# TXH-mercury/VALOR

Measured on AMD Instinct MI355X. Metric: pretrain samples/sec (V+A+T clip), higher is better.
Workload: dtype bf16

## Files before the change

valor_amd/csrc/gemm.hip:

```cpp
#include "gemm_common.h"
#include <stdlib.h>

template <typename T, bool TA, bool TB>
__global__ __launch_bounds__(256) void gemm_kernel(GemmArgs p) {
    constexpr int VEC = ElemTraits<T>::VEC;
    constexpr int BK = 8 * VEC;
    constexpr int TILE_BYTES = 128 * TILE_ROW_BYTES;
    extern __shared__ __attribute__((aligned(16))) char smem[];

    const int tid = threadIdx.x;
    const int lane = tid & 63;
    const int wave = __builtin_amdgcn_readfirstlane(tid >> 6);
    const int wm = wave >> 1, wn = wave & 1;

    const int tiles_n = (p.N + 127) >> 7;
    const int tiles_m = (p.M + 127) >> 7;
    const int logical = xcd_remap(blockIdx.x, tiles_m * tiles_n);
    const int tm = logical / tiles_n, tn = logical - tm * tiles_n;
    const int m0 = tm << 7, n0 = tn << 7;

    const int nk_total = (p.K + BK - 1) / BK;
    int ks_begin = 0, ks_end = nk_total;
    if (p.kslices > 1) {
        ks_begin = blockIdx.y * p.ksteps_per_slice;
// ... 329 lines not shown
    }
}

template <typename T>
DEVINL void splitk_reduce_body(const GemmArgs& p, int bid, int nblk) {
    if (p.ws_bf16 && (p.N & 7) == 0) {
        const int64_t noct = (int64_t)p.N >> 3, total8 = (int64_t)p.M * noct, sl = (int64_t)p.M * p.N;
        for (int64_t i = (int64_t)bid * blockDim.x + threadIdx.x; i < total8; i += (int64_t)nblk * blockDim.x) {
            const int m = (int)(i / noct);
            const int n = (int)(i - (int64_t)m * noct) << 3;
            const bf16_t* q = (const bf16_t*)p.ws + (int64_t)m * p.N + n;
            f32x4_t s0 = {0.f, 0.f, 0.f, 0.f}, s1 = s0;
            auto add = [&](const u32x4_t r) {
                s0 += (f32x4_t){__uint_as_float(r[0] << 16), __uint_as_float(r[0] & 0xffff0000u), __uint_as_float(r[1] << 16), __uint_as_float(r[1] & 0xffff0000u)};
                s1 += (f32x4_t){__uint_as_float(r[2] << 16), __uint_as_float(r[2] & 0xffff0000u), __uint_as_float(r[3] << 16), __uint_as_float(r[3] & 0xffff0000u)};
            };
            int k = 0;
            for (; k + 4 <= p.kslices; k += 4) {
                const u32x4_t r0 = *(const u32x4_t*)(q + (int64_t)k * sl), r1 = *(const u32x4_t*)(q + (int64_t)(k + 1) * sl);
                const u32x4_t r2 = *(const u32x4_t*)(q + (int64_t)(k + 2) * sl), r3 = *(const u32x4_t*)(q + (int64_t)(k + 3) * sl);
                add(r0); add(r1); add(r2); add(r3);
            }
            for (; k < p.kslices; ++k) add(*(const u32x4_t*)(q + (int64_t)k * sl));
            epilogue_store<T>(p, m, n, s0, load_bias4<T>(p, n));
            epilogue_store<T>(p, m, n + 4, s1, load_bias4<T>(p, n + 4));
        }
    } else {
    const int64_t nquads = ((int64_t)p.N + 3) >> 2;
    const int64_t total = (int64_t)p.M * nquads;
    for (int64_t i = (int64_t)bid * blockDim.x + threadIdx.x; i < total; i += (int64_t)nblk * blockDim.x) {
        const int m = (int)(i / nquads);
        const int n = (int)(i - (int64_t)m * nquads) << 2;
        f32x4_t s = {0.f, 0.f, 0.f, 0.f};
        if (p.ws_bf16) {
            for (int k = 0; k < p.kslices; ++k) {
                const bf16_t* q = (const bf16_t*)p.ws + ((int64_t)k * p.M + m) * p.N + n;
                if (n + 3 < p.N && (p.N & 3) == 0) s += load4<bf16_t>(q);
                else for (int r = 0; r < 4; ++r) if (n + r < p.N) s[r] += (float)q[r];
            }
        } else {
            for (int k = 0; k < p.kslices; ++k) {
                const float* q = p.ws + ((int64_t)k * p.M + m) * p.N + n;
                if (n + 3 < p.N && (p.N & 3) == 0) s += *(const f32x4_t*)q;
                else for (int r = 0; r < 4; ++r) if (n + r < p.N) s[r] += q[r];
            }
        }
        epilogue_store<T>(p, m, n, s, load_bias4<T>(p, n));
    }
    }
    if (p.rowsum_out) {
        for (int m = bid * blockDim.x + threadIdx.x; m < p.M; m += nblk * blockDim.x) {
            float t = 0.f;
            for (int k = 0; k < p.kslices; ++k) t += p.rowsum_ws[(int64_t)k * p.M + m];
            rowsum_store<T>(p, m, t);
        }
    }
}
template <typename T>
__global__ __launch_bounds__(256) void gemm_splitk_reduce(GemmArgs p) {
    splitk_reduce_body<T>(p, blockIdx.x, gridDim.x);
}

#define VALOR_REDUCE_GROUP 8
struct ReduceGroupArgs {
    GemmArgs g[VALOR_REDUCE_GROUP];
    int first[VALOR_REDUCE_GROUP + 1];
    int n;
};
template <typename T>
__global__ __launch_bounds__(256) void gemm_splitk_reduce_group(ReduceGroupArgs a) {
    int i = 0;
    while (i + 1 < a.n && (int)blockIdx.x >= a.first[i + 1]) ++i;
    splitk_reduce_body<T>(a.g[i], blockIdx.x - a.first[i], a.first[i + 1] - a.first[i]);
}
static int reduce_blocks(const GemmArgs& p) {
    const int64_t total = (int64_t)p.M * ((p.N + 3) / 4);
    int blocks = (int)((total + 255) / 256);
    return blocks > 4096 ? 4096 : blocks;
}

static int g_gemm_variant = 4;
static inline int gemm_variant() { return GEMM_KNOB(variant, g_gemm_variant); }
extern "C" int valor_gemm_set_variant(int v) { const int o = g_gemm_variant; if (v >= 0 && v <= 4) g_gemm_variant = v; return o; }
thread_local const GemmTuning* t_gemm_tuning = nullptr;
int g_gemm_policy_default[13] = {[] { const char* e = getenv("VALOR_GEMM_NT_MINK"); return e ? atoi(e) : 768; }(),
                        [] { const char* e = getenv("VALOR_GEMM_SPLITK_BF16"); return e ? atoi(e) : 1; }(),
                        [] { const char* e = getenv("VALOR_GEMM_MIN_TILES"); return e ? atoi(e) : 256; }(),
                        [] { const char* e = getenv("VALOR_GEMM_NT_MIN_TILES"); return e ? atoi(e) : 1024; }(),
                        [] { const char* e = getenv("VALOR_GEMM_RASTER"); return e ? atoi(e) : 1000; }(),
                        [] { const char* e = getenv("VALOR_GEMM_STORE"); return e ? atoi(e) : 1000; }(),
                        [] { const char* e = getenv("VALOR_GEMM_NTA"); return e ? atoi(e) : 0; }(),
                        [] { const char* e = getenv("VALOR_GEMM_NN_MINK"); return e ? atoi(e) : 128; }(),
                        [] { const char* e = getenv("VALOR_GEMM_NARROW"); return e ? atoi(e) : 1000; }(),
                        [] { const char* e = getenv("VALOR_GEMM_MFMA32"); return e ? atoi(e) : 0; }(),
                        [] { const char* e = getenv("VALOR_GEMM_WIDE"); return e ? atoi(e) : 0; }(),
                        [] { const char* e = getenv("VALOR_GEMM_SKINNY_ALL"); return e ? atoi(e) : 0; }(),
                        [] { const char* e = getenv("VALOR_GEMM_WAVE128"); return e ? atoi(e) : 1000; }()};
extern "C" int valor_gemm_set_policy(int key, int value) {
    if (key < 0 || key > 12) return VALOR_ERR_ARG;
    const int old = g_gemm_policy_default[key];
    if (value >= 0) g_gemm_policy_default[key] = value;
    return old;
}

static bool use_8ph(int dtype, int transA, int transB, int M, int N, int K, bool heavy_epi = false) {
    if (dtype != VALOR_DT_BF16 || gemm_variant() < 3) return false;
    if ((K % 64) != 0 || K < 128 || M < 256 || N < 256) return false;
    if (gemm_variant() == 3) return true;
    const int64_t tiles256 = (int64_t)((M + 255) / 256) * ((N + 255) / 256);
    if (transA && transB) return K >= 4096;
    if (!transA && !transB) return tiles256 >= gemm_policy(2) && K >= gemm_policy(7);
    if (!transA && transB) return tiles256 >= gemm_policy(3) && K >= (heavy_epi ? 1536 : gemm_policy(0));
    return false;
}

static bool use_8ph2(int dtype, int transA, int transB, int M, int N, int K, bool heavy_epi, bool big) {
    const int mode = gemm_policy(8);
    if (dtype != VALOR_DT_BF16 || gemm_variant() != 4 || mode == 0) return false;
    if ((K % 64) != 0 || K < 128 || M < 256 || N < 128) return false;
    if (transA && !transB) return false;
    if (mode == 1) return true;
    if (mode == 2) return !big;
    if (mode == 3) return big;
    (void)heavy_epi;
    if (transA) return false;
    if (!big) return true;
    const int64_t tiles256 = (int64_t)((M + 255) / 256) * ((N + 255) / 256);
    return K <= 1024 && (N >= 1536 || tiles256 < 1024);
}

static int gemm_family(int dtype, int transA, int transB, int M, int N, int K, bool heavy_epi) {
    if (dtype != VALOR_DT_BF16 || gemm_variant() == 0) return 0;
    if (gemm_variant() == 4 && !transA && !transB && M <= gemm_policy(11) && N >= 16 && gemm_skinny_chunks(K)) return 5;
    const bool big = use_8ph(dtype, transA, transB, M, N, K, heavy_epi);
    if (use_8ph2(dtype, transA, transB, M, N, K, heavy_epi, big)) return 4;
    if (big) return 3;
    return gemm_variant() == 2 ? 2 : 1;
}

static int family3_ktiles_per_workgroup(int M, int N, int K) {
    const int nk = K / 64, tiles = ((M + 255) / 256) * ((N + 255) / 256);
    int sl = 1;
    if (2 * tiles <= 256 && nk >= 24) {
        sl = 256 / tiles;
        if (sl > nk / 6) sl = nk / 6;
        if (sl > 64) sl = 64;
        if (sl < 2) sl = 1;
    }
    return (nk + sl - 1) / sl;
}
static bool use_wave128(int dtype, int transA, int transB, int M, int N, int K, bool heavy_epi) {
    const int mode = gemm_policy(12);
    if (mode == 0 || gemm_family(dtype, transA, transB, M, N, K, heavy_epi) != 3) return false;
    if (!(transA && transB)) return false;
    if (mode == 1) return true;
    return family3_ktiles_per_workgroup(M, N, K) > 48;
}
extern "C" int valor_gemm_wave128_for(int dtype, int transA, int transB, int M, int N, int K, int heavy_epilogue) {
    return use_wave128(dtype, transA, transB, M, N, K, heavy_epilogue != 0) ? 1 : 0;
}

extern "C" int valor_gemm_kernel_for(int dtype, int transA, int transB, int M, int N, int K, int heavy_epilogue) {
    return gemm_family(dtype, transA, transB, M, N, K, heavy_epilogue != 0);
}
struct TuningScope {
    const GemmTuning* prev;
    explicit TuningScope(const void* t) : prev(t_gemm_tuning) { if (t) t_gemm_tuning = (const GemmTuning*)t; }
    ~TuningScope() { t_gemm_tuning = prev; }
};
static_assert(sizeof(GemmTuning) == 17 * sizeof(int), "valor_gemm_policy layout (include/valor_hip.h)");
extern "C" int valor_gemm_kernel_for_tuned(const void* policy, int dtype, int transA, int transB, int M, int N, int K, int heavy_epilogue) {
    TuningScope scope(policy);
    return gemm_family(dtype, transA, transB, M, N, K, heavy_epilogue != 0);
}

template <int NSTAGE>
static void launch_gemm_glds(hipStream_t st, int transA, int transB, const GemmArgs& p, dim3 grid) {
    const size_t lds = NSTAGE * 32768;
#define VALOR_GLDS_LAUNCH1(TA_, TB_, F_, W_)                                                        \
    do {                                                                                            \
        static bool attr_set = false;                                                               \
        if (!attr_set) {                                                                            \
            hipFuncSetAttribute((const void*)gemm_glds_kernel<TA_, TB_, NSTAGE, F_, W_>,            \
                                hipFuncAttributeMaxDynamicSharedMemorySize, (int)lds);              \
            attr_set = true;                                                                        \
        }                                                                                           \
        hipLaunchKernelGGL((gemm_glds_kernel<TA_, TB_, NSTAGE, F_, W_>), grid, dim3(256), lds, st, p); \
    } while (0)
#define VALOR_GLDS_LAUNCH(TA_, TB_)                                                                 \
    do {                                                                                            \
        if constexpr (NSTAGE == 1) {                                                                \
            if (fused) VALOR_GLDS_LAUNCH1(TA_, TB_, true, 3);                                       \
            else VALOR_GLDS_LAUNCH1(TA_, TB_, false, 4);                                            \
        } else {                                                                                    \
            if (fused) VALOR_GLDS_LAUNCH1(TA_, TB_, true, 2);                                       \
            else VALOR_GLDS_LAUNCH1(TA_, TB_, false, 2);                                            \
        }                                                                                           \
    } while (0)
    const bool fused = p.kslices <= 1 && ((p.act & VALOR_ACT_MASK) != VALOR_ACT_NONE || p.preact || p.dact_aux);
    if (!transA && !transB) VALOR_GLDS_LAUNCH(false, false);
    else if (!transA && transB) VALOR_GLDS_LAUNCH(false, true);
    else if (transA && !transB) VALOR_GLDS_LAUNCH(true, false);
    else VALOR_GLDS_LAUNCH(true, true);
#undef VALOR_GLDS_LAUNCH
#undef VALOR_GLDS_LAUNCH1
}

template <typename T>
static int launch_gemm(hipStream_t st, int transA, int transB, GemmArgs p) {
    const int tiles = ((p.M + 127) / 128) * ((p.N + 127) / 128);
    dim3 grid(tiles, p.kslices > 1 ? p.kslices : 1);
    if (ElemTraits<T>::DT == VALOR_DT_BF16 && gemm_variant() > 0) {
        if (p.kslices > 1) grid = dim3(tiles * p.kslices, 1);
        const int fam = gemm_family(VALOR_DT_BF16, transA, transB, p.M, p.N, p.K, p.dact_aux != nullptr && !(p.act & VALOR_ACT_DERIV));
        if (fam == 4) launch_gemm_8ph2(st, transA, transB, p);
        else if (fam == 3) {
            if (use_wave128(VALOR_DT_BF16, transA, transB, p.M, p.N, p.K, p.dact_aux != nullptr && !(p.act & VALOR_ACT_DERIV))) launch_gemm_8q(st, transA, transB, p);
            else launch_gemm_8ph(st, transA, transB, p);
        } else {
            p.st_mode = (gemm_policy(6) && !p.out_f32 && p.kslices <= 1 && p.K <= 1024 && (int64_t)p.M * p.N >= (4 << 20)) ? 1 : 0;
            if (gemm_variant() == 2) launch_gemm_glds<2>(st, transA, transB, p, grid);
            else launch_gemm_glds<1>(st, transA, transB, p, grid);
        }
        if (p.kslices > 1 && !p.defer_reduce)
            hipLaunchKernelGGL((gemm_splitk_reduce<T>), dim3(reduce_blocks(p)), dim3(256), 0, st, p);
        return valor_launch_status();
    }
    const size_t lds = 2 * 2 * 128 * TILE_ROW_BYTES;
#define VALOR_GEMM_LAUNCH(TA_, TB_)                                                               \
    do {                                                                                          \
        static bool attr_set = false;                                                             \
        if (!attr_set) {                                                                          \
            hipFuncSetAttribute((const void*)gemm_kernel<T, TA_, TB_>,                            \
                                hipFuncAttributeMaxDynamicSharedMemorySize, (int)lds);            \
            attr_set = true;                                                                      \
        }                                                                                         \
        hipLaunchKernelGGL((gemm_kernel<T, TA_, TB_>), grid, dim3(256), lds, st, p);              \
    } while (0)
    if (!transA && !transB) VALOR_GEMM_LAUNCH(false, false);
    else if (!transA && transB) VALOR_GEMM_LAUNCH(false, true);
    else if (transA && !transB) VALOR_GEMM_LAUNCH(true, false);
    else VALOR_GEMM_LAUNCH(true, true);
#undef VALOR_GEMM_LAUNCH
    if (p.kslices > 1 && !p.defer_reduce)
        hipLaunchKernelGGL((gemm_splitk_reduce<T>), dim3(reduce_blocks(p)), dim3(256), 0, st, p);
    return valor_launch_status();
}

struct PendingBlob { GemmArgs p; int dtype; int valid; };
static_assert(sizeof(PendingBlob) <= 256, "valor_gemm_pending is 256 bytes");

static int gemm_impl(void* stream, int dtype, int transA, int transB, int M, int N, int K,
                     const void* A, int64_t lda, const void* B, int64_t ldb, void* C, int64_t ldc,
                     const void* bias, int act, void* preact, const void* dact_aux, int64_t ldaux,
                     float alpha, int accumulate, int out_f32, void* workspace, int64_t workspace_bytes,
                     void* rowsum_out, int rowsum_accumulate, PendingBlob* pending);

extern "C" int valor_gemm(void* stream, int dtype, int transA, int transB, int M, int N, int K,
                          const void* A, int64_t lda, const void* B, int64_t ldb, void* C, int64_t ldc,
                          const void* bias, int act, void* preact, const void* dact_aux, int64_t ldaux,
                          float alpha, int accumulate, int out_f32, void* workspace, int64_t workspace_bytes,
                          void* rowsum_out, int rowsum_accumulate) {
    return gemm_impl(stream, dtype, transA, transB, M, N, K, A, lda, B, ldb, C, ldc, bias, act, preact, dact_aux, ldaux, alpha, accumulate,
                     out_f32, workspace, workspace_bytes, rowsum_out, rowsum_accumulate, nullptr);
}

extern "C" int valor_gemm_tuned(const void* policy, void* stream, int dtype, int transA, int transB, int M, int N, int K,
                                const void* A, int64_t lda, const void* B, int64_t ldb, void* C, int64_t ldc,
                                const void* bias, int act, void* preact, const void* dact_aux, int64_t ldaux,
                                float alpha, int accumulate, int out_f32, void* workspace, int64_t workspace_bytes,
                                void* rowsum_out, int rowsum_accumulate) {
    TuningScope scope(policy);
    return gemm_impl(stream, dtype, transA, transB, M, N, K, A, lda, B, ldb, C, ldc, bias, act, preact, dact_aux, ldaux, alpha, accumulate,
                     out_f32, workspace, workspace_bytes, rowsum_out, rowsum_accumulate, nullptr);
}

extern "C" int valor_gemm_deferred(void* stream, int dtype, int transA, int transB, int M, int N, int K,
                                   const void* A, int64_t lda, const void* B, int64_t ldb, void* C, int64_t ldc,
                                   const void* bias, int act, void* preact, const void* dact_aux, int64_t ldaux,
                                   float alpha, int accumulate, int out_f32, void* workspace, int64_t workspace_bytes,
                                   void* rowsum_out, int rowsum_accumulate, void* pending) {
    if (!pending) return VALOR_ERR_ARG;
    PendingBlob* pb = (PendingBlob*)pending;
    pb->valid = 0; pb->dtype = dtype; pb->p.kslices = 0;
    return gemm_impl(stream, dtype, transA, transB, M, N, K, A, lda, B, ldb, C, ldc, bias, act, preact, dact_aux, ldaux, alpha, accumulate,
                     out_f32, workspace, workspace_bytes, rowsum_out, rowsum_accumulate, pb);
}

extern "C" int valor_gemm_pending_bytes(const void* pending, int64_t* bytes) {
    if (!pending || !bytes) return VALOR_ERR_ARG;
    const PendingBlob* pb = (const PendingBlob*)pending;
    *bytes = 0;
    if (!pb->valid || pb->p.kslices <= 1) return VALOR_OK;
    const int64_t n = ((int64_t)pb->p.kslices * pb->p.M * pb->p.N + (int64_t)pb->p.kslices * pb->p.M) * 4;
    *bytes = (n + 255) & ~(int64_t)255;
    return VALOR_OK;
}

extern "C" int valor_gemm_reduce_group(void* stream, int dtype, const void* pendings, int n) {
    if (n <= 0) return VALOR_OK;
    if (!pendings || n > VALOR_REDUCE_GROUP) return VALOR_ERR_ARG;
    ReduceGroupArgs a;
    a.n = 0; a.first[0] = 0;
    for (int i = 0; i < n; ++i) {
        const PendingBlob* pb = (const PendingBlob*)((const char*)pendings + (size_t)i * 256);
        if (!pb->valid || pb->p.kslices <= 1) continue;
        if (pb->dtype != dtype) return VALOR_ERR_ARG;
        a.g[a.n] = pb->p;
// ... 123 lines not shown
```

valor_amd/csrc/gemm8.hip:

```cpp
#include "gemm_common.h"
#include <stdlib.h>

#define HT_BYTES 16384
#define BUF_BYTES (4 * HT_BYTES)
#define OFF_A0 0
#define OFF_A1 HT_BYTES
#define OFF_B0 (2 * HT_BYTES)
#define OFF_B1 (3 * HT_BYTES)

DEVINL bf16x8_t read_frag_tr8(const char* img, int off, int kk) {
    const char* a = img + off + kk * (32 * 256);
    s16x4_t lo = lds_read_tr4(a), hi = lds_read_tr4(a + 4 * 256);
    return __builtin_bit_cast(bf16x8_t, __builtin_shufflevector(lo, hi, 0, 1, 2, 3, 4, 5, 6, 7));
}

template <bool TA, bool TB, bool ASMTR, bool NTS = false, int SCHED = 0>
__global__ __launch_bounds__(512, 2) void gemm_8ph_kernel(GemmArgs p) {
    typedef bf16_t T;
    constexpr int BK = 64;
    extern __shared__ __attribute__((aligned(16))) char smem[];

    const int tid = threadIdx.x;
    const int lane = tid & 63;
    const int wave = __builtin_amdgcn_readfirstlane(tid >> 6);
// ... 349 lines not shown
        }
    }

    if constexpr (!TA) if (p.fast_epi) {
        char* sB = smem;
        const int act = p.act & VALOR_ACT_MASK;
        const bool deriv = (p.act & VALOR_ACT_DERIV) != 0;
        auto write_tile = [&](bool apply_act) {
#pragma unroll
            for (int ni = 0; ni < 4; ++ni) {
                const int col = (ni >> 1) * 128 + wn * 32 + (ni & 1) * 16 + 4 * fg;
                const f32x4_t bias4 = load_bias4<T>(p, n0 + col);
#pragma unroll
                for (int mi = 0; mi < 8; ++mi) {
                    const int row = (mi >> 2) * 128 + wm * 64 + (mi & 3) * 16 + fr;
                    f32x4_t v = acc[mi][ni];
#pragma unroll
                    for (int r = 0; r < 4; ++r) v[r] = v[r] * p.alpha + bias4[r];
                    if (apply_act) {
                        float f[4] = {v[0], v[1], v[2], v[3]};
                        act_fwd_n<4>(act, f);
                        v = (f32x4_t){f[0], f[1], f[2], f[3]};
                    }
                    const u32x2_t w = {pack2_bf16(v[0], v[1]), pack2_bf16(v[2], v[3])};
                    *(u32x2_t*)(sB + row * 512 + (((col >> 3) ^ (row & 31)) << 4) + (fg & 1) * 8) = w;
                }
            }
        };
        auto read_tile = [&](T* dst) {
#pragma unroll 4
            for (int it = 0; it < 16; ++it) {
                const int ml = it * 16 + (tid >> 5), c = tid & 31;
                const u32x4_t val = *(const u32x4_t*)(sB + ml * 512 + ((c ^ (ml & 31)) << 4));
                const int m = m0 + ml, n = n0 + c * 8;
                if (m < p.M && n < p.N) store_out16<NTS>(dst + (int64_t)m * p.ldc + n, val);
            }
        };
        if (p.preact) {
            write_tile(false);
            __syncthreads();
            read_tile((T*)p.preact);
            __syncthreads();
        }
        write_tile(act != VALOR_ACT_NONE && !p.dact_aux);
        if (p.dact_aux || p.accumulate) {
            const bool dact = p.dact_aux != nullptr, accum = p.accumulate != 0;
            const T* src = dact ? (const T*)p.dact_aux : (const T*)p.C;
            const int64_t lds2 = dact ? p.ldaux : p.ldc;
            u32x4_t pre[16];
#pragma unroll
            for (int it = 0; it < 16; ++it) {
                const int m = m0 + it * 16 + (tid >> 5), n = n0 + (tid & 31) * 8;
                pre[it] = (u32x4_t){0u, 0u, 0u, 0u};
                if (m < p.M && n < p.N) pre[it] = *(const u32x4_t*)(src + (int64_t)m * lds2 + n);
            }
            __syncthreads();
            T* dst = (T*)p.C;
#pragma unroll
            for (int it = 0; it < 16; ++it) {
                const int ml = it * 16 + (tid >> 5), c = tid & 31;
                u32x4_t val = *(const u32x4_t*)(sB + ml * 512 + ((c ^ (ml & 31)) << 4));
                const int m = m0 + ml, n = n0 + c * 8;
                if (m < p.M && n < p.N) {
                    float f[8], x[8];
#pragma unroll
                    for (int q = 0; q < 4; ++q) { f[2 * q] = __uint_as_float(val[q] << 16); f[2 * q + 1] = __uint_as_float(val[q] & 0xffff0000u); }
#pragma unroll
                    for (int q = 0; q < 4; ++q) { x[2 * q] = __uint_as_float(pre[it][q] << 16); x[2 * q + 1] = __uint_as_float(pre[it][q] & 0xffff0000u); }
                    if (dact) {
                        if (deriv) {
#pragma unroll
                            for (int q = 0; q < 8; ++q) f[q] *= x[q];
                        } else {
                            act_bwd_mul_n<8>(act, f, x);
                        }
                        if (accum) {
                            const u32x4_t o = *(const u32x4_t*)(dst + (int64_t)m * p.ldc + n);
#pragma unroll
                            for (int q = 0; q < 4; ++q) { f[2 * q] += __uint_as_float(o[q] << 16); f[2 * q + 1] += __uint_as_float(o[q] & 0xffff0000u); }
                        }
                    } else {
#pragma unroll
                        for (int q = 0; q < 8; ++q) f[q] += x[q];
                    }
#pragma unroll
                    for (int q = 0; q < 4; ++q) val[q] = pack2_bf16(f[2 * q], f[2 * q + 1]);
                    store_out16<NTS>(dst + (int64_t)m * p.ldc + n, val);
                }
            }
            return;
        }
        __syncthreads();
        read_tile((T*)p.C);
        return;
    }

    float* sC = (float*)smem;
    float* wsl = p.kslices > 1 ? p.ws + (int64_t)slice * p.M * p.N : nullptr;
    const f32x4_t bias0 = load_bias4<T>(p, n0 + (tid & 31) * 8), bias1 = load_bias4<T>(p, n0 + (tid & 31) * 8 + 4);
#pragma unroll
    for (int pass = 0; pass < 2; ++pass) {
        if (pass) __syncthreads();
#pragma unroll
        for (int mt = 0; mt < 4; ++mt)
#pragma unroll
            for (int ni = 0; ni < 4; ++ni) {
                const int ml = wm * 64 + mt * 16 + fr;
                const int ch = ((ni >> 1) * 32 + wn * 8 + (ni & 1) * 4 + fg) ^ (ml & 7);
                *(f32x4_t*)(sC + ml * 256 + ch * 4) = acc[pass * 4 + mt][ni];
            }
        __syncthreads();
#pragma unroll 2
        for (int it = 0; it < 8; ++it) {
            const int ml = it * 16 + (tid >> 5);
            const int c8 = tid & 31;
            const f32x4_t v0 = *(const f32x4_t*)(sC + ml * 256 + (((2 * c8) ^ (ml & 7)) << 2));
            const f32x4_t v1 = *(const f32x4_t*)(sC + ml * 256 + (((2 * c8 + 1) ^ (ml & 7)) << 2));
            const int m = m0 + pass * 128 + ml, n = n0 + c8 * 8;
            if (wsl) {
                splitk_store8(p, slice, m, n, v0, v1);
            } else {
                epilogue_store8<true, NTS ? 1 : 0>(p, m, n, v0, v1, bias0, bias1);
            }
        }
    }
}

static int g_8ph_tr_asm = [] { const char* e = getenv("VALOR_GEMM_TR_ASM"); return e ? atoi(e) : 1; }();
extern "C" int valor_gemm_set_tr_asm(int v) {
    const int old = g_8ph_tr_asm;
    if (v >= 0) g_8ph_tr_asm = v;
    return old;
}

static int g_8ph_fast_epi = [] { const char* e = getenv("VALOR_GEMM_FAST_EPI"); return e ? atoi(e) : 1; }();
extern "C" int valor_gemm_set_fast_epilogue(int v) {
    const int old = g_8ph_fast_epi;
    if (v >= 0) g_8ph_fast_epi = v;
    return old;
}

static int g_8ph_sched = [] { const char* e = getenv("VALOR_GEMM_8PH_SCHED"); return e ? atoi(e) : 1000; }();
extern "C" int valor_gemm_set_8ph_sched(int v) {
    const int old = g_8ph_sched;
    if (v == 0 || v == 1 || v == 1000) g_8ph_sched = v;
    return old;
}

int gemm_tr_asm_now() { return GEMM_KNOB(tr_asm, g_8ph_tr_asm); }
int gemm_fast_epilogue_now() { return GEMM_KNOB(fast_epilogue, g_8ph_fast_epi); }

void launch_gemm_8ph(hipStream_t st, int transA, int transB, const GemmArgs& p_in) {
    GemmArgs p = p_in;
    const int fast_epi_ = gemm_fast_epilogue_now(), tr_asm_ = gemm_tr_asm_now();
    const bool light_dact = p.dact_aux && (p.act & VALOR_ACT_DERIV);
    const bool plainish = fast_epi_ >= 2 || (!p.preact && (!p.dact_aux || light_dact));
    p.fast_epi = fast_epi_ && plainish && !p.out_f32 && p.kslices <= 1 && (p.N & 7) == 0 && (p.ldc & 7) == 0 && !p.rowsum_out &&
                 (!p.dact_aux || (p.ldaux & 7) == 0) && !(p.dact_aux && p.preact) && !transA && !(p.preact && (p.act & VALOR_ACT_DERIV));
    const int tiles_m = (p.M + 255) / 256, tiles_n = (p.N + 255) / 256;
    const int tiles = tiles_m * tiles_n;
    p.raster_g = 0;
    if (p.kslices <= 1 && tiles_n > 1 && gemm_policy(4) != 0) {
        if (gemm_policy(4) != 1000) {
            p.raster_g = gemm_policy(4) < tiles_n ? gemm_policy(4) : 0;
        } else {
            const double panel = 256.0 * p.K * 2.0, a_bytes = (double)p.M * p.K * 2.0, rounds = tiles / 256.0;
            const double resident = 2.5 * 1048576.0;
            const int touched = tiles_n < 32 ? tiles_n : 32;
            double best = a_bytes + (tiles_n * panel <= resident ? 8.0 * tiles_n * panel : (rounds < 1.0 ? 1.0 : rounds) * 8.0 * touched * panel);
            for (int ng = 2; ng <= tiles_n; ++ng) {
                const int G = (tiles_n + ng - 1) / ng;
                if (G * panel > resident) continue;
                const double cost = ng * a_bytes + 8.0 * tiles_n * panel;
                if (cost < 0.9 * best) { best = cost; p.raster_g = G; }
            }
        }
    }
    const bool nts = !transA && !p.out_f32 && p.kslices <= 1 && (gemm_policy(5) == 1 || (gemm_policy(5) == 1000 && p.K <= 1024));
    p.st_mode = nts ? 1 : 0;
    dim3 grid(tiles * (p.kslices > 1 ? p.kslices : 1));
    const size_t lds = 2 * BUF_BYTES;
    int sched = GEMM_KNOB(sched_256, g_8ph_sched);
    if (sched == 1000) {
        const int ktiles = p.kslices > 1 ? p.ksteps_per_slice : p.K / 64;
        sched = transA ? (ktiles <= 48 ? 1 : 0) : (p.K >= 2048 ? 1 : 0);
    }
#define VALOR_8PH_LAUNCH(TA_, TB_, NTS_)                                                                        \
    do {                                                                                                        \
        static bool attr_set = false;                                                                           \
        constexpr bool kslow_ = TA_ || TB_;                                                                     \
        if (!attr_set) {                                                                                        \
            hipFuncSetAttribute((const void*)gemm_8ph_kernel<TA_, TB_, false, NTS_>, hipFuncAttributeMaxDynamicSharedMemorySize, (int)lds); \
            hipFuncSetAttribute((const void*)gemm_8ph_kernel<TA_, TB_, true, NTS_>, hipFuncAttributeMaxDynamicSharedMemorySize, (int)lds); \
            hipFuncSetAttribute((const void*)gemm_8ph_kernel<TA_, TB_, kslow_, NTS_, 1>, hipFuncAttributeMaxDynamicSharedMemorySize, (int)lds); \
            attr_set = true;                                                                                    \
        }                                                                                                       \
        if (sched == 1 && (tr_asm_ || !kslow_)) hipLaunchKernelGGL((gemm_8ph_kernel<TA_, TB_, kslow_, NTS_, 1>), grid, dim3(512), lds, st, p); \
        else if (tr_asm_ && kslow_) hipLaunchKernelGGL((gemm_8ph_kernel<TA_, TB_, true, NTS_>), grid, dim3(512), lds, st, p); \
        else hipLaunchKernelGGL((gemm_8ph_kernel<TA_, TB_, false, NTS_>), grid, dim3(512), lds, st, p);       \
    } while (0)
    if (!transA && !transB) { if (nts) VALOR_8PH_LAUNCH(false, false, true); else VALOR_8PH_LAUNCH(false, false, false); }
    else if (!transA && transB) { if (nts) VALOR_8PH_LAUNCH(false, true, true); else VALOR_8PH_LAUNCH(false, true, false); }
    else if (transA && !transB) VALOR_8PH_LAUNCH(true, false, false);
    else VALOR_8PH_LAUNCH(true, true, false);
#undef VALOR_8PH_LAUNCH
}
```

valor_amd/csrc/gemm8q.hip:

```cpp
#include "gemm_common.h"
#include <stdlib.h>

#define HT_BYTES 16384
#define BUF_BYTES (4 * HT_BYTES)
#define OFF_A0 0
#define OFF_A1 HT_BYTES
#define OFF_B0 (2 * HT_BYTES)
#define OFF_B1 (3 * HT_BYTES)

template <bool KSLOW> struct FragSet;
template <> struct FragSet<false> { bf16x8_t f[4][2]; };
template <> struct FragSet<true> { TrPair f[4][2]; };
DEVINL bf16x8_t frag_of(const bf16x8_t& f) { return f; }
DEVINL bf16x8_t frag_of(const TrPair& t) { return tr_frag(t); }
DEVINL void mfma_acc(f32x4_t& c, bf16x8_t a, bf16x8_t b) { asm("v_mfma_f32_16x16x32_bf16 %0, %1, %2, %0" : "+a"(c) : "v"(a), "v"(b)); }
DEVINL void mfma_rowsum(f32x4_t& r0, f32x4_t& r1, bf16x8_t ones, bf16x8_t f0, bf16x8_t f1, bf16x8_t f2, bf16x8_t f3, int sel) {
    asm volatile("s_cmp_lt_i32 %7, 1\n\ts_cbranch_scc1 2f\n\ts_cmp_eq_u32 %7, 1\n\ts_cbranch_scc0 1f\n\t"
                 "v_mfma_f32_16x16x32_bf16 %0, %2, %3, %0\n\tv_mfma_f32_16x16x32_bf16 %1, %2, %4, %1\n\ts_branch 2f\n"
                 "1:\n\tv_mfma_f32_16x16x32_bf16 %0, %2, %5, %0\n\tv_mfma_f32_16x16x32_bf16 %1, %2, %6, %1\n"
                 "2:"
                 : "+v"(r0), "+v"(r1) : "v"(ones), "v"(f0), "v"(f1), "v"(f2), "v"(f3), "s"(sel) : "scc");
}
DEVINL void wait8(FragSet<false>&) { asm volatile("s_waitcnt lgkmcnt(0)" ::: "memory"); }
DEVINL void wait8(FragSet<true>& s) { tr_wait8(s.f); }
// ... 78 lines not shown
                    oA[hf][i] = (k_first + k) * ldA_b + (m0 + hf * 128 + ic) * 2;
                }
                if constexpr (!TB) {
                    const int r = pc * 8 + (lane >> 3), c = (lane & 7) ^ ((lane >> 3) & 7);
                    oB[hf][i] = (n0 + hf * 128 + r) * ldB_b + (k_first + c * 8) * 2;
                } else {
                    const int k = pc * 4 + (lane >> 4), s = lane & 15;
                    const int ic = ((s - 2 * (k & 3) - 8 * ((k >> 3) & 1)) & 15) * 8;
                    oB[hf][i] = (k_first + k) * ldB_b + (n0 + hf * 128 + ic) * 2;
                }
            }
        stepA = TA ? BK * ldA_b : BK * 2;
        stepB = TB ? BK * ldB_b : BK * 2;
    }
    auto dmaA = [&](int hf, char* buf, int t, int i) {
        const rsrc_t rs = make_rsrc(p.A, t < ntile ? p.bytesA : 0u);
        glds16(rs, buf + (hf ? OFF_A1 : OFF_A0) + wave * 4096 + i * 1024, oA[hf][i]);
        oA[hf][i] += stepA; asm volatile("" : "+v"(oA[hf][i]));
    };
    auto dmaB = [&](int hf, char* buf, int t, int i) {
        const rsrc_t rs = make_rsrc(p.B, t < ntile ? p.bytesB : 0u);
        glds16(rs, buf + (hf ? OFF_B1 : OFF_B0) + wave * 4096 + i * 1024, oB[hf][i]);
        oB[hf][i] += stepB; asm volatile("" : "+v"(oB[hf][i]));
    };

    int trA[4], trB[4];
    {
        const int base = (8 * fg + (fr >> 2)) * 256 + 8 * (fr & 1);
        const int rot = 2 * (fr >> 2) + 8 * (fg & 1);
#pragma unroll
        for (int i = 0; i < 4; ++i) {
            trA[i] = base + 16 * ((2 * (wm * 4 + i) + ((fr >> 1) & 1) + rot) & 15);
            trB[i] = base + 16 * ((2 * (wn * 4 + i) + ((fr >> 1) & 1) + rot) & 15);
        }
    }
    auto rdA = [&](const char* img, FragSet<TA>& s, int mt, int kk) {
        if constexpr (TA) tr_issue(s.f[mt][kk], img + trA[mt] + kk * (32 * 256));
        else s.f[mt][kk] = read_frag<T>(img, wm * 64 + mt * 16 + fr, kk * 4 + fg);
    };
    auto rdB = [&](const char* img, FragSet<TB>& s, int nt, int kk) {
        if constexpr (TB) tr_issue(s.f[nt][kk], img + trB[nt] + kk * (32 * 256));
        else s.f[nt][kk] = read_frag<T>(img, wn * 64 + nt * 16 + fr, kk * 4 + fg);
    };
#define PIN() __builtin_amdgcn_sched_barrier(0)
    auto quadrant = [&](int mh, int nh, FragSet<TA>& sa, FragSet<TB>& sb, auto&& slot) __attribute__((always_inline)) {
#pragma unroll
        for (int kk = 0; kk < 2; ++kk)
#pragma unroll
            for (int mt = 0; mt < 4; ++mt)
#pragma unroll
                for (int nt = 0; nt < 4; ++nt) {
                    const int i = kk * 16 + mt * 4 + nt;
                    mfma_acc(acc[mh * 4 + mt][nh * 4 + nt], frag_of(sb.f[nt][kk]), frag_of(sa.f[mt][kk]));
                    slot(i);
                    PIN();
                }
    };
    auto rowsum = [&](int hh, FragSet<TA>& sa) __attribute__((always_inline)) {
        if constexpr (TA) {
#pragma unroll
            for (int kk = 0; kk < 2; ++kk)
                mfma_rowsum(racc[hh][0], racc[hh][1], ones, frag_of(sa.f[0][kk]), frag_of(sa.f[1][kk]), frag_of(sa.f[2][kk]), frag_of(sa.f[3][kk]), rs_sel);
            PIN();
        }
    };
#define PHASE_END()                                                                                               \
    do {                                                                                                          \
        asm volatile("s_waitcnt vmcnt(20)" ::: "memory");                                                         \
        __builtin_amdgcn_s_barrier();                                                                             \
        PIN();                                                                                                    \
    } while (0)

    FragSet<TA> fax, fay;
    FragSet<TB> fb0, fb1;
    if (ntile > 0) {
#pragma unroll
        for (int t = 0; t < 2; ++t) {
            char* const b = smem + t * BUF_BYTES;
#pragma unroll
            for (int i = 0; i < 4; ++i) dmaA(0, b, t, i);
#pragma unroll
            for (int i = 0; i < 4; ++i) dmaB(0, b, t, i);
#pragma unroll
            for (int i = 0; i < 4; ++i) dmaB(1, b, t, i);
#pragma unroll
            for (int i = 0; i < 4; ++i) dmaA(1, b, t, i);
        }
        PIN();
        PHASE_END();
#pragma unroll
        for (int i = 0; i < 8; ++i) rdA(smem + OFF_A0, fax, i & 3, i >> 2);
#pragma unroll
        for (int i = 0; i < 4; ++i) rdB(smem + OFF_B0, fb0, i, 0);
        PIN();
        wait8(fax); wait4(fb0, 0);
        __builtin_amdgcn_s_barrier();
        PIN();
        for (int rel = 0; rel < ntile; ++rel) {
            char* const cur = smem + (rel & 1) * BUF_BYTES;
            char* const nxt = smem + ((rel & 1) ^ 1) * BUF_BYTES;
            quadrant(0, 0, fax, fb0, [&](int i) {
                if (i < 4) rdB(cur + OFF_B0, fb0, i, 1);
                else if (i < 8) dmaA(0, cur, rel + 2, i - 4);
                else if (i == 15) { PIN(); wait4(fb0, 1); }
                else if (i >= 16 && i < 24) rdB(cur + OFF_B1, fb1, i & 3, (i - 16) >> 2);
            });
            rowsum(0, fax);
            PIN();
            wait8(fb1);
            PHASE_END();
            quadrant(0, 1, fax, fb1, [&](int i) {
                if (i < 8) rdA(cur + OFF_A1, fay, i & 3, i >> 2);
                else if (i < 16 && !(i & 1)) dmaB(0, cur, rel + 2, (i - 8) >> 1);
            });
            PIN();
            wait8(fay);
            PHASE_END();
            quadrant(1, 1, fay, fb1, [&](int i) {
                if (i < 4) rdA(nxt + OFF_A0, fax, i, 0);
                else if (i >= 8 && i < 16 && !(i & 1)) dmaB(1, cur, rel + 2, (i - 8) >> 1);
            });
            rowsum(1, fay);
            PIN();
            wait4(fax, 0);
            PHASE_END();
            quadrant(1, 0, fay, fb0, [&](int i) {
                if (i < 4) rdA(nxt + OFF_A0, fax, i, 1);
                else if (i >= 8 && i < 16 && !(i & 1)) dmaA(1, cur, rel + 2, (i - 8) >> 1);
                else if (i >= 16 && i < 20) rdB(nxt + OFF_B0, fb0, i - 16, 0);
            });
            PIN();
            wait4(fax, 1); wait4(fb0, 0);
            PHASE_END();
        }
    }
    asm volatile("s_nop 15\n\ts_nop 15\n\ts_waitcnt vmcnt(0)" ::: "memory");
    PIN();
    __syncthreads();
#undef PHASE_END
#undef PIN
    if (do_rs && fg == 0) {
#pragma unroll
        for (int hh = 0; hh < 2; ++hh)
#pragma unroll
            for (int i = 0; i < 2; ++i) {
                const int m = m0 + hh * 128 + wm * 64 + (2 * wn + i) * 16 + fr;
                if (m < p.M) {
                    if (p.kslices > 1) p.rowsum_ws[(int64_t)slice * p.M + m] = racc[hh][i][0];
                    else rowsum_store<T>(p, m, racc[hh][i][0]);
                }
            }
    }

    float* sC = (float*)smem;
    float* wsl = p.kslices > 1 ? p.ws + (int64_t)slice * p.M * p.N : nullptr;
    const f32x4_t bias0 = load_bias4<T>(p, n0 + (tid & 31) * 8), bias1 = load_bias4<T>(p, n0 + (tid & 31) * 8 + 4);
#pragma unroll
    for (int pass = 0; pass < 2; ++pass) {
        if (pass) __syncthreads();
#pragma unroll
        for (int mt = 0; mt < 4; ++mt)
#pragma unroll
            for (int ni = 0; ni < 8; ++ni) {
                const int ml = wm * 64 + mt * 16 + fr;
                const int ch = ((ni >> 2) * 32 + wn * 16 + (ni & 3) * 4 + fg) ^ (ml & 7);
                *(f32x4_t*)(sC + ml * 256 + ch * 4) = acc[pass * 4 + mt][ni];
            }
        __syncthreads();
#pragma unroll 2
        for (int it = 0; it < 16; ++it) {
            const int ml = it * 8 + (tid >> 5);
            const int c8 = tid & 31;
            const f32x4_t v0 = *(const f32x4_t*)(sC + ml * 256 + (((2 * c8) ^ (ml & 7)) << 2));
            const f32x4_t v1 = *(const f32x4_t*)(sC + ml * 256 + (((2 * c8 + 1) ^ (ml & 7)) << 2));
            const int m = m0 + pass * 128 + ml, n = n0 + c8 * 8;
            if (wsl) {
                splitk_store8(p, slice, m, n, v0, v1);
            } else {
                epilogue_store8<true, 0>(p, m, n, v0, v1, bias0, bias1);
            }
        }
    }
}

void launch_gemm_8q(hipStream_t st, int transA, int transB, const GemmArgs& p_in) {
    GemmArgs p = p_in;
    p.fast_epi = 0;
    p.raster_g = 0;
    p.st_mode = 0;
    const int tiles = ((p.M + 255) / 256) * ((p.N + 255) / 256);
    dim3 grid(tiles * (p.kslices > 1 ? p.kslices : 1));
    const size_t lds = 2 * BUF_BYTES;
#define VALOR_8Q_LAUNCH(TA_, TB_)                                                                               \
    do {                                                                                                        \
        static bool attr_set = false;                                                                           \
        if (!attr_set) {                                                                                        \
            hipFuncSetAttribute((const void*)gemm_8q_kernel<TA_, TB_>, hipFuncAttributeMaxDynamicSharedMemorySize, (int)lds); \
            attr_set = true;                                                                                    \
        }                                                                                                       \
        hipLaunchKernelGGL((gemm_8q_kernel<TA_, TB_>), grid, dim3(256), lds, st, p);                            \
    } while (0)
    if (transA && transB) VALOR_8Q_LAUNCH(true, true);
    else if (!transA && !transB) VALOR_8Q_LAUNCH(false, false);
    else if (!transA && transB) VALOR_8Q_LAUNCH(false, true);
    else VALOR_8Q_LAUNCH(true, false);
#undef VALOR_8Q_LAUNCH
}
```

valor_amd/csrc/gemm_common.h:

```cpp
#pragma once
#include "mma.h"

struct GemmArgs {
    const void* A; const void* B; void* C;
    const void* bias;
    void* preact;
    const void* dact_aux;
    float* ws;
    int64_t lda, ldb, ldc, ldaux;
    int M, N, K;
    int act;
    int accumulate;
    int out_f32;
    int kslices;
    int ksteps_per_slice;
    float alpha;
    uint32_t bytesA, bytesB;
    void* rowsum_out;
    float* rowsum_ws;
    int rowsum_acc;
    int fast_epi;
    int raster_g;
    int st_mode;
    int ws_bf16;
// ... 46 lines not shown
        *o = (p.rowsum_acc ? *o : 0.f) + v;
    } else {
        T* o = (T*)p.rowsum_out + m;
        *o = from_f32<T>((p.rowsum_acc ? to_f32<T>(*o) : 0.f) + v);
    }
}

template <typename T, bool FUSED = true>
DEVINL void epilogue_store(const GemmArgs& p, int m, int n0, f32x4_t acc, f32x4_t bias4) {
    if (m >= p.M || n0 >= p.N) return;
    const int nvalid = p.N - n0 < 4 ? p.N - n0 : 4;
    const int64_t off = (int64_t)m * p.ldc + n0;
    const bool vec = nvalid == 4 && ((p.ldc & 3) == 0);
    f32x4_t v;
#pragma unroll
    for (int r = 0; r < 4; ++r) v[r] = acc[r] * p.alpha + bias4[r];
    if constexpr (FUSED) {
        const int act = p.act & VALOR_ACT_MASK;
        const bool deriv = (p.act & VALOR_ACT_DERIV) != 0;
        f32x4_t pre = v;
        if ((act != VALOR_ACT_NONE || (deriv && p.preact)) && !p.dact_aux) {
            float f[4] = {v[0], v[1], v[2], v[3]};
            if (p.preact && deriv) {
                float g[4];
                act_fwd_deriv_n<4>(act, f, g);
                pre = (f32x4_t){g[0], g[1], g[2], g[3]};
            } else {
                act_fwd_n<4>(act, f);
            }
            v = (f32x4_t){f[0], f[1], f[2], f[3]};
        }
        if (p.preact) {
            if (p.out_f32) {
                float* q = (float*)p.preact + off;
                if (vec) *(f32x4_t*)q = pre;
                else for (int r = 0; r < nvalid; ++r) q[r] = pre[r];
            } else {
                T* q = (T*)p.preact + off;
                if (vec) store4<T>(q, pre);
                else for (int r = 0; r < nvalid; ++r) q[r] = from_f32<T>(pre[r]);
            }
        }
        if (p.dact_aux) {
            const T* a = (const T*)p.dact_aux + (int64_t)m * p.ldaux + n0;
            if (vec && (p.ldaux & 3) == 0) {
                const f32x4_t u = load4<T>(a);
                if (deriv) {
                    v *= u;
                } else {
                    float f[4] = {v[0], v[1], v[2], v[3]};
                    const float x[4] = {u[0], u[1], u[2], u[3]};
                    act_bwd_mul_n<4>(act, f, x);
                    v = (f32x4_t){f[0], f[1], f[2], f[3]};
                }
            } else {
                for (int r = 0; r < nvalid; ++r) v[r] *= deriv ? to_f32<T>(a[r]) : act_bwd(act, to_f32<T>(a[r]));
            }
        }
    }
    if (p.out_f32) {
        float* c = (float*)p.C + off;
        if (vec) {
            if (p.accumulate) { f32x4_t o = *(f32x4_t*)c; v += o; }
            *(f32x4_t*)c = v;
        } else {
            for (int r = 0; r < nvalid; ++r) c[r] = (p.accumulate ? c[r] : 0.f) + v[r];
        }
    } else {
        T* c = (T*)p.C + off;
        if (vec) {
            if (p.accumulate) { f32x4_t o = load4<T>(c); v += o; }
            store4<T>(c, v);
        } else {
            for (int r = 0; r < nvalid; ++r)
                c[r] = from_f32<T>((p.accumulate ? to_f32<T>(c[r]) : 0.f) + v[r]);
        }
    }
}


template <bool FUSED = true, int NTS = -1>
DEVINL void epilogue_store8(const GemmArgs& p, int m, int n0, f32x4_t a0, f32x4_t a1, f32x4_t b0, f32x4_t b1) {
    typedef bf16_t T;
    if (m >= p.M || n0 >= p.N) return;
    const bool vec8 = n0 + 8 <= p.N && (p.ldc & 7) == 0 && !p.out_f32 && (!p.dact_aux || (p.ldaux & 7) == 0);
    if (!vec8) {
        epilogue_store<T, FUSED>(p, m, n0, a0, b0);
        epilogue_store<T, FUSED>(p, m, n0 + 4, a1, b1);
        return;
    }
    const int64_t off = (int64_t)m * p.ldc + n0;
    f32x4_t v0, v1;
#pragma unroll
    for (int r = 0; r < 4; ++r) { v0[r] = a0[r] * p.alpha + b0[r]; v1[r] = a1[r] * p.alpha + b1[r]; }
    if constexpr (FUSED) {
        const int act = p.act & VALOR_ACT_MASK;
        const bool deriv = (p.act & VALOR_ACT_DERIV) != 0;
        f32x4_t q0 = v0, q1 = v1;
        if ((act != VALOR_ACT_NONE || (deriv && p.preact)) && !p.dact_aux) {
            float f[8] = {v0[0], v0[1], v0[2], v0[3], v1[0], v1[1], v1[2], v1[3]};
            if (p.preact && deriv) {
                float g[8];
                act_fwd_deriv_n<8>(act, f, g);
                q0 = (f32x4_t){g[0], g[1], g[2], g[3]};
                q1 = (f32x4_t){g[4], g[5], g[6], g[7]};
            } else {
                act_fwd_n<8>(act, f);
            }
            v0 = (f32x4_t){f[0], f[1], f[2], f[3]};
            v1 = (f32x4_t){f[4], f[5], f[6], f[7]};
        }
        if (p.preact) {
            u32x4_t q = {pack2_bf16(q0[0], q0[1]), pack2_bf16(q0[2], q0[3]), pack2_bf16(q1[0], q1[1]), pack2_bf16(q1[2], q1[3])};
            if constexpr (NTS < 0) store_out16(p.st_mode, (T*)p.preact + off, q);
            else store_out16<NTS != 0>((T*)p.preact + off, q);
        }
        if (p.dact_aux) {
            const T* a = (const T*)p.dact_aux + (int64_t)m * p.ldaux + n0;
            const f32x4_t u0 = load4<T>(a), u1 = load4<T>(a + 4);
            if (deriv) {
                v0 *= u0; v1 *= u1;
            } else {
                float f[8] = {v0[0], v0[1], v0[2], v0[3], v1[0], v1[1], v1[2], v1[3]};
                const float x[8] = {u0[0], u0[1], u0[2], u0[3], u1[0], u1[1], u1[2], u1[3]};
                act_bwd_mul_n<8>(act, f, x);
                v0 = (f32x4_t){f[0], f[1], f[2], f[3]};
                v1 = (f32x4_t){f[4], f[5], f[6], f[7]};
            }
        }
    }
    T* c = (T*)p.C + off;
    if (p.accumulate) { v0 += load4<T>(c); v1 += load4<T>(c + 4); }
    u32x4_t o = {pack2_bf16(v0[0], v0[1]), pack2_bf16(v0[2], v0[3]), pack2_bf16(v1[0], v1[1]), pack2_bf16(v1[2], v1[3])};
    if constexpr (NTS < 0) store_out16(p.st_mode, c, o);
    else store_out16<NTS != 0>(c, o);
}

void launch_gemm_8ph(hipStream_t st, int transA, int transB, const GemmArgs& p);
void launch_gemm_8q(hipStream_t st, int transA, int transB, const GemmArgs& p);
void launch_gemm_8ph2(hipStream_t st, int transA, int transB, const GemmArgs& p);
void launch_gemm_8w(hipStream_t st, const GemmArgs& p, int tiles, bool nts);
int gemm_skinny_chunks(int K);
int launch_gemm_skinny(hipStream_t st, const GemmArgs& p);
struct GemmTuning { int key[12]; int variant, tr_asm, fast_epilogue, sched_256, sched_narrow; };
extern thread_local const GemmTuning* t_gemm_tuning;
extern int g_gemm_policy_default[13];
static inline int gemm_policy(int k) {
    const GemmTuning* o = t_gemm_tuning;
    return (o && k < 12 && o->key[k] >= 0) ? o->key[k] : g_gemm_policy_default[k];
}
#define GEMM_KNOB(FIELD_, GLOBAL_) ((t_gemm_tuning && t_gemm_tuning->FIELD_ >= 0) ? t_gemm_tuning->FIELD_ : (GLOBAL_))
int gemm_tr_asm_now();
int gemm_fast_epilogue_now();
```

Measured before the change: 576.3.

## Add fast bf16 LDS-staged epilogue to 8q GEMM and share 256-tile planning

Moves the fast-epilogue, raster-group and non-temporal-store planning into a shared plan_256 helper. The 8q kernel now uses it too, where before it forced these off. For non-transposed A, the 8q kernel gains a fast epilogue: it applies bias and activation in registers, stages bf16 results through swizzled LDS, prefetches any dact/accumulate operand, and writes 16-byte rows. Preact cases fall back to the 8ph kernel. The wave128 forced mode now also applies to non-TA/TB shapes. The new path adds register pressure (32-entry prefetch array) and code-path complexity.

```diff
diff --git a/valor_amd/csrc/gemm.hip b/valor_amd/csrc/gemm.hip
--- a/valor_amd/csrc/gemm.hip
+++ b/valor_amd/csrc/gemm.hip
@@ -505,8 +505,8 @@
 static bool use_wave128(int dtype, int transA, int transB, int M, int N, int K, bool heavy_epi) {
     const int mode = gemm_policy(12);
     if (mode == 0 || gemm_family(dtype, transA, transB, M, N, K, heavy_epi) != 3) return false;
+    if (mode == 1) return true;
     if (!(transA && transB)) return false;
-    if (mode == 1) return true;
     return family3_ktiles_per_workgroup(M, N, K) > 48;
 }
 extern "C" int valor_gemm_wave128_for(int dtype, int transA, int transB, int M, int N, int K, int heavy_epilogue) {
diff --git a/valor_amd/csrc/gemm8.hip b/valor_amd/csrc/gemm8.hip
--- a/valor_amd/csrc/gemm8.hip
+++ b/valor_amd/csrc/gemm8.hip
@@ -525,32 +525,10 @@
 
 void launch_gemm_8ph(hipStream_t st, int transA, int transB, const GemmArgs& p_in) {
     GemmArgs p = p_in;
-    const int fast_epi_ = gemm_fast_epilogue_now(), tr_asm_ = gemm_tr_asm_now();
-    const bool light_dact = p.dact_aux && (p.act & VALOR_ACT_DERIV);
-    const bool plainish = fast_epi_ >= 2 || (!p.preact && (!p.dact_aux || light_dact));
-    p.fast_epi = fast_epi_ && plainish && !p.out_f32 && p.kslices <= 1 && (p.N & 7) == 0 && (p.ldc & 7) == 0 && !p.rowsum_out &&
-                 (!p.dact_aux || (p.ldaux & 7) == 0) && !(p.dact_aux && p.preact) && !transA && !(p.preact && (p.act & VALOR_ACT_DERIV));
-    const int tiles_m = (p.M + 255) / 256, tiles_n = (p.N + 255) / 256;
-    const int tiles = tiles_m * tiles_n;
-    p.raster_g = 0;
-    if (p.kslices <= 1 && tiles_n > 1 && gemm_policy(4) != 0) {
-        if (gemm_policy(4) != 1000) {
-            p.raster_g = gemm_policy(4) < tiles_n ? gemm_policy(4) : 0;
-        } else {
-            const double panel = 256.0 * p.K * 2.0, a_bytes = (double)p.M * p.K * 2.0, rounds = tiles / 256.0;
-            const double resident = 2.5 * 1048576.0;
-            const int touched = tiles_n < 32 ? tiles_n : 32;
-            double best = a_bytes + (tiles_n * panel <= resident ? 8.0 * tiles_n * panel : (rounds < 1.0 ? 1.0 : rounds) * 8.0 * touched * panel);
-            for (int ng = 2; ng <= tiles_n; ++ng) {
-                const int G = (tiles_n + ng - 1) / ng;
-                if (G * panel > resident) continue;
-                const double cost = ng * a_bytes + 8.0 * tiles_n * panel;
-                if (cost < 0.9 * best) { best = cost; p.raster_g = G; }
-            }
-        }
-    }
-    const bool nts = !transA && !p.out_f32 && p.kslices <= 1 && (gemm_policy(5) == 1 || (gemm_policy(5) == 1000 && p.K <= 1024));
-    p.st_mode = nts ? 1 : 0;
+    const int tr_asm_ = gemm_tr_asm_now();
+    plan_256(p, transA);
+    const bool nts = p.st_mode != 0;
+    const int tiles = ((p.M + 255) / 256) * ((p.N + 255) / 256);
     dim3 grid(tiles * (p.kslices > 1 ? p.kslices : 1));
     const size_t lds = 2 * BUF_BYTES;
     int sched = GEMM_KNOB(sched_256, g_8ph_sched);
diff --git a/valor_amd/csrc/gemm8q.hip b/valor_amd/csrc/gemm8q.hip
--- a/valor_amd/csrc/gemm8q.hip
+++ b/valor_amd/csrc/gemm8q.hip
@@ -254,9 +254,101 @@
             }
     }
 
+    if constexpr (!TA) if (p.fast_epi) {
+        char* sB = smem;
+        int et = tid;
+        asm volatile("" : "+v"(et));
+        const int efr = et & 15, efg = (et >> 4) & 3, erow = et >> 5, ec = et & 31;
+        const int act = p.act & VALOR_ACT_MASK;
+        const bool deriv = (p.act & VALOR_ACT_DERIV) != 0;
+        const bool dact = p.dact_aux != nullptr, accum = p.accumulate != 0;
+        const bool second = dact || accum;
+        T* dst = (T*)p.C;
+        f32x4_t bias4[8];
+#pragma unroll
+        for (int ni = 0; ni < 8; ++ni) bias4[ni] = load_bias4<T>(p, n0 + (ni >> 2) * 128 + wn * 64 + (ni & 3) * 16 + 4 * efg);
+        const bool apply_act = act != VALOR_ACT_NONE && !dact;
+#pragma unroll
+        for (int ni = 0; ni < 8; ++ni) {
+            const int col = (ni >> 2) * 128 + wn * 64 + (ni & 3) * 16 + 4 * efg;
+#pragma unroll
+            for (int mi = 0; mi < 8; ++mi) {
+                const int row = (mi >> 2) * 128 + wm * 64 + (mi & 3) * 16 + efr;
+                f32x4_t v = acc[mi][ni];
+#pragma unroll
+                for (int r = 0; r < 4; ++r) v[r] = v[r] * p.alpha + bias4[ni][r];
+                if (apply_act) {
+                    float f[4] = {v[0], v[1], v[2], v[3]};
+                    act_fwd_n<4>(act, f);
+                    v = (f32x4_t){f[0], f[1], f[2], f[3]};
+                }
+                const u32x2_t w = {pack2_bf16(v[0], v[1]), pack2_bf16(v[2], v[3])};
+                *(u32x2_t*)(sB + row * 512 + (((col >> 3) ^ (row & 31)) << 4) + (efg & 1) * 8) = w;
+            }
+        }
+        u32x4_t pre[32];
+        if (second) {
+            const T* src = dact ? (const T*)p.dact_aux : (const T*)p.C;
+            const int64_t lds2 = dact ? p.ldaux : p.ldc;
+#pragma unroll
+            for (int it = 0; it < 32; ++it) {
+                const int m = m0 + it * 8 + erow, n = n0 + ec * 8;
+                pre[it] = (u32x4_t){0u, 0u, 0u, 0u};
+                if (m < p.M && n < p.N) pre[it] = *(const u32x4_t*)(src + (int64_t)m * lds2 + n);
+            }
+        }
+        __syncthreads();
+        if (second) {
+#pragma unroll
+            for (int it = 0; it < 32; ++it) {
+                const int ml = it * 8 + erow, c = ec;
+                u32x4_t val = *(const u32x4_t*)(sB + ml * 512 + ((c ^ (ml & 31)) << 4));
+                const int m = m0 + ml, n = n0 + c * 8;
+                if (m < p.M && n < p.N) {
+                    float f[8], x[8];
+#pragma unroll
+                    for (int q = 0; q < 4; ++q) { f[2 * q] = __uint_as_float(val[q] << 16); f[2 * q + 1] = __uint_as_float(val[q] & 0xffff0000u); }
+#pragma unroll
+                    for (int q = 0; q < 4; ++q) { x[2 * q] = __uint_as_float(pre[it][q] << 16); x[2 * q + 1] = __uint_as_float(pre[it][q] & 0xffff0000u); }
+                    if (dact) {
+                        if (deriv) {
+#pragma unroll
+                            for (int q = 0; q < 8; ++q) f[q] *= x[q];
+                        } else {
+                            act_bwd_mul_n<8>(act, f, x);
+                        }
+                        if (accum) {
+                            const u32x4_t o = *(const u32x4_t*)(dst + (int64_t)m * p.ldc + n);
+#pragma unroll
+                            for (int q = 0; q < 4; ++q) { f[2 * q] += __uint_as_float(o[q] << 16); f[2 * q + 1] += __uint_as_float(o[q] & 0xffff0000u); }
+                        }
+                    } else {
+#pragma unroll
+                        for (int q = 0; q < 8; ++q) f[q] += x[q];
+                    }
+#pragma unroll
+                    for (int q = 0; q < 4; ++q) val[q] = pack2_bf16(f[2 * q], f[2 * q + 1]);
+                    store_out16(p.st_mode, dst + (int64_t)m * p.ldc + n, val);
+                }
+            }
+            return;
+        }
+#pragma unroll 4
+        for (int it = 0; it < 32; ++it) {
+            const int ml = it * 8 + erow, c = ec;
+            const u32x4_t val = *(const u32x4_t*)(sB + ml * 512 + ((c ^ (ml & 31)) << 4));
+            const int m = m0 + ml, n = n0 + c * 8;
+            if (m < p.M && n < p.N) store_out16(p.st_mode, dst + (int64_t)m * p.ldc + n, val);
+        }
+        return;
+    }
+
     float* sC = (float*)smem;
+    int gt = tid;
+    if constexpr (!TA) asm volatile("" : "+v"(gt));
+    const int gfr = TA ? fr : (gt & 15), gfg = TA ? fg : ((gt >> 4) & 3);
     float* wsl = p.kslices > 1 ? p.ws + (int64_t)slice * p.M * p.N : nullptr;
-    const f32x4_t bias0 = load_bias4<T>(p, n0 + (tid & 31) * 8), bias1 = load_bias4<T>(p, n0 + (tid & 31) * 8 + 4);
+    const f32x4_t bias0 = load_bias4<T>(p, n0 + (gt & 31) * 8), bias1 = load_bias4<T>(p, n0 + (gt & 31) * 8 + 4);
 #pragma unroll
     for (int pass = 0; pass < 2; ++pass) {
         if (pass) __syncthreads();
@@ -264,22 +356,22 @@
         for (int mt = 0; mt < 4; ++mt)
 #pragma unroll
             for (int ni = 0; ni < 8; ++ni) {
-                const int ml = wm * 64 + mt * 16 + fr;
-                const int ch = ((ni >> 2) * 32 + wn * 16 + (ni & 3) * 4 + fg) ^ (ml & 7);
+                const int ml = wm * 64 + mt * 16 + gfr;
+                const int ch = ((ni >> 2) * 32 + wn * 16 + (ni & 3) * 4 + gfg) ^ (ml & 7);
                 *(f32x4_t*)(sC + ml * 256 + ch * 4) = acc[pass * 4 + mt][ni];
             }
         __syncthreads();
 #pragma unroll 2
         for (int it = 0; it < 16; ++it) {
-            const int ml = it * 8 + (tid >> 5);
-            const int c8 = tid & 31;
+            const int ml = it * 8 + (gt >> 5);
+            const int c8 = gt & 31;
             const f32x4_t v0 = *(const f32x4_t*)(sC + ml * 256 + (((2 * c8) ^ (ml & 7)) << 2));
             const f32x4_t v1 = *(const f32x4_t*)(sC + ml * 256 + (((2 * c8 + 1) ^ (ml & 7)) << 2));
             const int m = m0 + pass * 128 + ml, n = n0 + c8 * 8;
             if (wsl) {
                 splitk_store8(p, slice, m, n, v0, v1);
             } else {
-                epilogue_store8<true, 0>(p, m, n, v0, v1, bias0, bias1);
+                epilogue_store8<true, TA ? 0 : -1>(p, m, n, v0, v1, bias0, bias1);
             }
         }
     }
@@ -287,9 +379,8 @@
 
 void launch_gemm_8q(hipStream_t st, int transA, int transB, const GemmArgs& p_in) {
     GemmArgs p = p_in;
-    p.fast_epi = 0;
-    p.raster_g = 0;
-    p.st_mode = 0;
+    plan_256(p, transA);
+    if (p.preact && p.fast_epi) { launch_gemm_8ph(st, transA, transB, p_in); return; }
     const int tiles = ((p.M + 255) / 256) * ((p.N + 255) / 256);
     dim3 grid(tiles * (p.kslices > 1 ? p.kslices : 1));
     const size_t lds = 2 * BUF_BYTES;
diff --git a/valor_amd/csrc/gemm_common.h b/valor_amd/csrc/gemm_common.h
--- a/valor_amd/csrc/gemm_common.h
+++ b/valor_amd/csrc/gemm_common.h
@@ -222,3 +222,32 @@
 #define GEMM_KNOB(FIELD_, GLOBAL_) ((t_gemm_tuning && t_gemm_tuning->FIELD_ >= 0) ? t_gemm_tuning->FIELD_ : (GLOBAL_))
 int gemm_tr_asm_now();
 int gemm_fast_epilogue_now();
+
+static inline void plan_256(GemmArgs& p, int transA) {
+    const int fast_epi_ = gemm_fast_epilogue_now();
+    const bool light_dact = p.dact_aux && (p.act & VALOR_ACT_DERIV);
+    const bool plainish = fast_epi_ >= 2 || (!p.preact && (!p.dact_aux || light_dact));
+    p.fast_epi = fast_epi_ && plainish && !p.out_f32 && p.kslices <= 1 && (p.N & 7) == 0 && (p.ldc & 7) == 0 && !p.rowsum_out &&
+                 (!p.dact_aux || (p.ldaux & 7) == 0) && !(p.dact_aux && p.preact) && !transA && !(p.preact && (p.act & VALOR_ACT_DERIV));
+    const int tiles_m = (p.M + 255) / 256, tiles_n = (p.N + 255) / 256;
+    const int tiles = tiles_m * tiles_n;
+    p.raster_g = 0;
+    if (p.kslices <= 1 && tiles_n > 1 && gemm_policy(4) != 0) {
+        if (gemm_policy(4) != 1000) {
+            p.raster_g = gemm_policy(4) < tiles_n ? gemm_policy(4) : 0;
+        } else {
+            const double panel = 256.0 * p.K * 2.0, a_bytes = (double)p.M * p.K * 2.0, rounds = tiles / 256.0;
+            const double resident = 2.5 * 1048576.0;
+            const int touched = tiles_n < 32 ? tiles_n : 32;
+            double best = a_bytes + (tiles_n * panel <= resident ? 8.0 * tiles_n * panel : (rounds < 1.0 ? 1.0 : rounds) * 8.0 * touched * panel);
+            for (int ng = 2; ng <= tiles_n; ++ng) {
+                const int G = (tiles_n + ng - 1) / ng;
+                if (G * panel > resident) continue;
+                const double cost = ng * a_bytes + 8.0 * tiles_n * panel;
+                if (cost < 0.9 * best) { best = cost; p.raster_g = G; }
+            }
+        }
+    }
+    const bool nts = !transA && !p.out_f32 && p.kslices <= 1 && (gemm_policy(5) == 1 || (gemm_policy(5) == 1000 && p.K <= 1024));
+    p.st_mode = nts ? 1 : 0;
+}
```

New measurement: 577.2, median of 2. Within noise of the previous version (+0.2%).
